# facebookresearch/dmc-net

Hardware: AMD Instinct MI355X
Metric: clips/sec (3-seg 224x224) DMC-gen+ResNet-18 train step (higher is better)
Workload: dtype f32

## Files before the change

dmc-net_amd/csrc/conv_x3q.hip:

```cpp
#include "dmc_common.h"
#include "x3s_common.h"
#include <type_traits>
#include <utility>

using namespace dmc;
using namespace dmc::x3;

namespace {

constexpr int QBM = 256, QBN = 64;
constexpr int QWSLOT = 3 * QBN * 32;
constexpr int QWB = 3 * QWSLOT;
constexpr int QEP = 272, QETILE = 32 * QEP;

template <int NW_, int NPB_, int NT_>
struct QG {
    static constexpr int NW = NW_, NPB = NPB_, NT = NT_;
    static constexpr int NA = NW / 2;
    static constexpr int KP = (NT + NA - 1) / NA;
    static constexpr int PT = 3 * KP;
    static constexpr int KW = (18 + NA - 1) / NA;
    static constexpr int ZROW = 32 * NT;
    static constexpr int PSL = (ZROW + 1) * 32;
    static constexpr int PB = 3 * PSL;
// ... 129 lines not shown
#pragma unroll
        for (int j = 0; j < TN; ++j)
#pragma unroll
            for (int e = 0; e < 16; ++e) acc[s][j][e] = 0.f;

    lds_cptr const L = (lds_cptr)lds_q;
    struct Frag { u32x4 X[3], W[TN][3]; };
    auto load_frags = [&](Frag& f, int xa, int wa, auto kc) {
        constexpr int k = decltype(kc)::value;
#pragma unroll
        for (int s = 0; s < 3; ++s) {
#pragma unroll
            for (int j = 0; j < TN; ++j)
                f.W[j][s] = *reinterpret_cast<const __attribute__((address_space(3))) u32x4*>(L + wa + ((k * 3 + s) * QBN + 32 * j) * 32);
            f.X[s] = *reinterpret_cast<const __attribute__((address_space(3))) u32x4*>(L + xa + s * QPSL);
        }
    };
    auto mfma_slot = [&](const Frag& f, auto ac, auto&& between) {
        constexpr int A = decltype(ac)::value;
#pragma unroll
        for (int p = 0; p < 6; ++p) {
            constexpr int WS[6] = {0, 0, 0, 1, 1, 2}, XS[6] = {2, 1, 0, 1, 0, 0};
#pragma unroll
            for (int j = 0; j < TN; ++j) acc[A][j] = mfma_bf16(f.W[j][WS[p]], f.X[XS[p]], acc[A][j]);
            between(p);
        }
    };
    auto nothing = [](int) {};
    constexpr int NRD = 3 + 3 * TN, NMF = 6 * TN;
    auto interleave = [&]() {
#pragma unroll
        for (int k = 0; k < (NRD < NMF ? NRD : NMF); ++k) {
            __builtin_amdgcn_sched_group_barrier(0x008, 1, 0);
            __builtin_amdgcn_sched_group_barrier(0x100, 1, 0);
        }
        if constexpr (NMF > NRD) __builtin_amdgcn_sched_group_barrier(0x008, NMF - NRD, 0);
    };

    if (tid < 2 * 3 * QNPB)
        *reinterpret_cast<float4*>(lds_q + (tid >> 1) / 3 * QPB + ((tid >> 1) % 3) * QPSL + QZROW * 32 + (tid & 1) * 16) = make_float4(0.f, 0.f, 0.f, 0.f);
    if (grp_a) {
        static_for<QNPB>([&](auto uc) {
            constexpr int U = decltype(uc)::value;
            if (U < total_units) {
#pragma unroll
                for (int i = 0; i < QPT; ++i) dma_patch(U / NUNIT, std::integral_constant<int, U % NUNIT>{}, U, i);
            }
// ... 54 lines not shown
            constexpr int kl = nslot - 1;
            constexpr int sh_first = P::STEP[JN].s[0].sh, acc_last = P::STEP[J].s[kl].acc;
            if (g + 1 < total_steps)
                load_frags(frag_of(std::integral_constant<int, (par + kl + 1) & 1>{}), xcur[sh_first], wcur, std::integral_constant<int, 0>{});
            constexpr int J2 = (J + 2) % NSTEP, C2 = (J + 2) / NSTEP;
            constexpr int U3 = (unit + QNPB) % NUNIT, CU3 = (unit + QNPB) / NUNIT;
            const bool wgo = !grp_a && g + 2 < total_steps;
            const bool pgo = grp_a && unit_last && U + QNPB < total_units;
            mfma_slot(frag_of(std::integral_constant<int, (par + kl) & 1>{}), std::integral_constant<int, acc_last>{}, [&](int p) {
                if (wgo) {
#pragma unroll
                    for (int i = p; i < KW; i += 6) dma_weight(c + C2, std::integral_constant<int, J2>{}, wb_old, wq + NA * i);
                }
                if constexpr (unit_last) {
                    if (pgo) {
#pragma unroll
                        for (int i = p; i < QPT; i += 6) dma_patch(c + CU3, std::integral_constant<int, U3>{}, pb_old, i);
                    }
                }
            });
        });
    }

    __syncthreads();
    constexpr int CW = 32 * TN, LPR = CW / 4, RPI = 64 / LPR;
    char* etile = lds_q + wave * QETILE;
    const int mw0 = m0 + wm * 32;
    const int rbase = blockIdx.y * QBN + wn * CW;
    const bool ok = mw0 + l31 <= mlast;
#pragma unroll
    for (int A = 0; A < NACC; ++A) {
#pragma unroll
        for (int j = 0; j < TN; ++j)
#pragma unroll
            for (int g4 = 0; g4 < 4; ++g4) {
                float4 v = make_float4(acc[A][j][4 * g4], acc[A][j][4 * g4 + 1], acc[A][j][4 * g4 + 2], acc[A][j][4 * g4 + 3]);
                if (!ok) v = make_float4(0.f, 0.f, 0.f, 0.f);
                *reinterpret_cast<float4*>(etile + l31 * QEP + (32 * j + 8 * g4 + 4 * khalf) * 4) = v;
            }
        float* const yout = (NACC == 2 && A == 1) ? a.y1 : a.y0;
        if constexpr (EVAL) {
            const int c4 = rbase + (lane % LPR) * 4;
            const float* const st = A == 1 ? a.stats1 : a.stats0;
            const float4 mean = *reinterpret_cast<const float4*>(st + c4), istd = *reinterpret_cast<const float4*>(st + a.R + c4);
            const float4 gm = *reinterpret_cast<const float4*>((A == 1 ? a.gamma1 : a.gamma0) + c4);
            const float4 bt = *reinterpret_cast<const float4*>((A == 1 ? a.beta1 : a.beta0) + c4);
            unsigned short* const ys = A == 1 ? nullptr : a.ys0;
#pragma unroll
            for (int it = 0; it < 32 / RPI; ++it) {
                const int prow = RPI * it + lane / LPR;
                const int m = mw0 + prow;
                const float4 v = *reinterpret_cast<const float4*>(etile + prow * QEP + (lane % LPR) * 16);
                if (m <= mlast) {
                    const float w[4] = {bn_apply_act1(v.x, mean.x, istd.x, gm.x, bt.x, false, 0.f, A == 0),
                                        bn_apply_act1(v.y, mean.y, istd.y, gm.y, bt.y, false, 0.f, A == 0),
                                        bn_apply_act1(v.z, mean.z, istd.z, gm.z, bt.z, false, 0.f, A == 0),
                                        bn_apply_act1(v.w, mean.w, istd.w, gm.w, bt.w, false, 0.f, A == 0)};
                    if (yout) *reinterpret_cast<float4*>(yout + (size_t)m * a.R + c4) = make_float4(w[0], w[1], w[2], w[3]);
                    if (ys) x3s_store4(ys, w, (size_t)a.M, a.R >> 4, (size_t)m, c4 >> 2);
                }
            }
        } else {
#pragma unroll
        for (int it = 0; it < 32 / RPI; ++it) {
            const int prow = RPI * it + lane / LPR;
            const int m = mw0 + prow;
            const float4 v = *reinterpret_cast<const float4*>(etile + prow * QEP + (lane % LPR) * 16);
            if (m <= mlast) {
                size_t opix = (size_t)m;
                if (NACC == 4) {
                    const int n = m / HW, rem = m - n * HW, ya = rem / a.W, xb = rem - ya * a.W;
                    opix = ((size_t)n * (2 * a.H) + 2 * ya + (A >> 1)) * (2 * a.W) + 2 * xb + (A & 1);
                }
                *reinterpret_cast<float4*>(yout + opix * a.R + rbase + (lane % LPR) * 4) = v;
            }
        }
        }
        if (NACC == 2 && !EVAL) {
            double* const part = A == 1 ? a.part1 : a.part0;
            if (part) {
                double* red = reinterpret_cast<double*>(lds_q + QNW * QETILE);
                if (lane < CW) {
                    double d1 = 0.0, d2 = 0.0;
#pragma unroll 8
                    for (int p = 0; p < 32; ++p) {
                        const double v = (double)*reinterpret_cast<const float*>(etile + p * QEP + lane * 4);
                        d1 += v;
                        d2 += v * v;
                    }
                    red[(wm * 64 + wn * CW + lane) * 2 + 0] = d1;
                    red[(wm * 64 + wn * CW + lane) * 2 + 1] = d2;
                }
                __syncthreads();
                for (int cc = tid; cc < QBN; cc += QNW * 64) {
                    double e1 = 0.0, e2 = 0.0;
#pragma unroll
                    for (int w = 0; w < WM; ++w) { e1 += red[(w * 64 + cc) * 2 + 0]; e2 += red[(w * 64 + cc) * 2 + 1]; }
                    double* dst = part + ((size_t)blockIdx.x * a.R + blockIdx.y * QBN + cc) * 2;
                    dst[0] = e1; dst[1] = e2;
                }
                __syncthreads();
            }
        }
    }
}

__global__ __launch_bounds__(256) void x3q_pack_w_kernel(const float* __restrict__ w3, const float* __restrict__ w1,
                                                         unsigned short* __restrict__ wf, unsigned short* __restrict__ wt, int Cout, int Cin) {
    const bool transposed = blockIdx.y == 1;
    unsigned short* dst = transposed ? wt : wf;
    if (!dst) return;
    const int R = transposed ? Cin : Cout, K = transposed ? Cout : Cin;
    const int nchunk = K >> 4;
    const long total = (long)R * 10 * K;
    for (long i = (long)blockIdx.x * 256 + threadIdx.x; i < total; i += (long)gridDim.x * 256) {
        long t = i;
        const int kk = (int)(t & 15); t >>= 4;
        const int rl = (int)(t & 63); t >>= 6;
        const int slot = (int)(t % 10); t /= 10;
        const int ch = (int)(t % nchunk);
        const int rt = (int)(t / nchunk);
        const int r = rt * 64 + rl, k = ch * 16 + kk;
        constexpr int FWD_TAP[10] = {0, 2, 6, 8, 3, 5, 1, 7, 4, 9};
        const int tap = transposed ? slot : FWD_TAP[slot];
// ... 550 lines not shown
```

dmc-net_amd/csrc/conv_x3s.hip:

```cpp
#include "dmc_common.h"
#include "x3s_common.h"
#include <type_traits>

using namespace dmc;
using namespace dmc::x3;

namespace {

__global__ __launch_bounds__(256) void x3s_split_kernel(const float* __restrict__ x, unsigned short* __restrict__ xs, long M, int C) {
    const int c8 = C >> 3;
    const long total = M * c8;
    const int nchunk = C >> 4;
    for (long o = (long)blockIdx.x * 256 + threadIdx.x; o < total; o += (long)gridDim.x * 256) {
        const long m = o / c8;
        const int g = (int)(o - m * c8);
        const float4 a = reinterpret_cast<const float4*>(x)[2 * o], b = reinterpret_cast<const float4*>(x)[2 * o + 1];
        const float v[8] = {a.x, a.y, a.z, a.w, b.x, b.y, b.z, b.w};
        x3s_store8(xs, v, (size_t)M, nchunk, (size_t)m, g);
    }
}

__global__ __launch_bounds__(256) void x3s_merge_kernel(const unsigned short* __restrict__ xs, float* __restrict__ x, long M, int C) {
    const long total = M * C;
    const size_t plane = (size_t)M * 16;
// ... 50 lines not shown
    const float* bnb_beta = nullptr;
    const unsigned char* bnb_mask = nullptr;
    int bnb_relu = 0;
    double* bnb_part = nullptr;
    int part_blocks = -1;
    int ablate;
    int bms = 0;
};
struct X3EvalArgs : X3Args {
    const float* stats;
    const float* gamma;
    const float* beta;
    const float* res;
    unsigned short* ys;
    int s2d, relu;
};

template <int WM, int WN, int TM, int TN, int PPMAX, bool STAG = false, int CLS = 1, bool EVAL = false, bool ROWT = false>
__global__ __launch_bounds__(WM * WN * 64) void x3s_conv_kernel(std::conditional_t<EVAL, X3EvalArgs, X3Args> a) {
    static_assert(!EVAL || CLS == 1, "the eval epilogue belongs to the forward convolution");
    static_assert(!ROWT || CLS == 1, "row-aligned tiles: forward and stride-1 data gradient");
    constexpr int NW = WM * WN, BM = 32 * TM * WM, BN = 32 * TN * WN;
    static_assert(BN == 64, "packed weight image is 64 rows wide");
    static_assert(PPMAX % 32 == 0 || PPMAX % 32 == 1, "patch transfers move 32 pixel rows");
    constexpr int PSL = PPMAX * 32;
    constexpr int PB = 3 * PSL;
    constexpr int WB = 3 * 3 * BN * 32;
    constexpr int WOFF = 2 * PB;
    static_assert(!STAG || NW >= 4, "two transfer groups need four waves");
    constexpr int NA = STAG ? NW / 2 : NW, NB = NW - (STAG ? NA : 0);
    constexpr int NDW = (PPMAX / 32 + NA - 1) / NA;
    constexpr int NEW = WB / 1024;
    constexpr int NEWW = (NEW + NB - 1) / NB;
    extern __shared__ __attribute__((aligned(1024))) char lds_x3[];

    const int tid = threadIdx.x, lane = tid & 63;
    const int wave = __builtin_amdgcn_readfirstlane(tid >> 6);
    const int wm = wave % WM, wn = wave / WM;
    const int l31 = lane & 31, khalf = lane >> 5;
    const unsigned lds0 = lds_addr_of(lds_x3);

    const int HW = a.H * a.W, PW = a.W;
    constexpr int ZROW = PPMAX - 1;
    const int bms = ROWT ? a.bms : BM;
    const int m0 = blockIdx.x * bms;
    const int mlast = (m0 + bms < a.M ? m0 + bms : a.M) - 1;
// ... 73 lines not shown
            xa[i] = xaddr[i][t];
            if constexpr (ROWT && pbuf == 1) asm volatile("" : "+v"(xa[i]));
        }
#pragma unroll
        for (int s = 0; s < 3; ++s) {
#pragma unroll
            for (int j = 0; j < TN; ++j)
                f.W[j][s] = *reinterpret_cast<const __attribute__((address_space(3))) u32x4*>(
                    L + waddr + (WOFF + wbuf * WB + (((t % 3) * 3 + s) * BN + 32 * j) * 32));
#pragma unroll
            for (int i = 0; i < TM; ++i)
                f.X[i][s] = *reinterpret_cast<const __attribute__((address_space(3))) u32x4*>(L + xa[i] + (pbuf * PB + s * PSL));
        }
    };
    auto mfma_frags = [&](const Frag& f, auto tc, auto&& between) {
        constexpr int t = decltype(tc)::value;
        constexpr int cl = CLS == 4 ? (t / 3 != 1) * 2 + (t % 3 != 1) : 0;
#pragma unroll
        for (int p = 0; p < 6; ++p) {
            constexpr int WS[6] = {0, 0, 0, 1, 1, 2}, XS[6] = {2, 1, 0, 1, 0, 0};
#pragma unroll
            for (int i = 0; i < TM; ++i)
#pragma unroll
                for (int j = 0; j < TN; ++j) acc[cl][i][j] = mfma_bf16(f.W[j][WS[p]], f.X[i][XS[p]], acc[cl][i][j]);
            between(p);
        }
    };
    auto nothing = [](int) {};
    constexpr int NRD = 3 * (TM + TN), NMF = 6 * TM * TN;
    auto interleave = [&]() {
#pragma unroll
        for (int k = 0; k < NRD; ++k) {
            __builtin_amdgcn_sched_group_barrier(0x008, 1, 0);
            __builtin_amdgcn_sched_group_barrier(0x100, 1, 0);
        }
        __builtin_amdgcn_sched_group_barrier(0x008, NMF - NRD, 0);
    };
    const bool dma_on = !(DMC_ABL(a.ablate) & 64);
    auto step = [&](auto pbufc, auto wbufc, auto qc, Frag& FA, Frag& FB, int c) {
        constexpr int pbuf = decltype(pbufc)::value, wbuf = decltype(wbufc)::value, q = decltype(qc)::value;
        using NP = std::integral_constant<int, q == 2 ? (pbuf ^ 1) : pbuf>;
        using NWB = std::integral_constant<int, wbuf ^ 1>;
        using NT = std::integral_constant<int, q == 2 ? 0 : 3 * (q + 1)>;
        using T0 = std::integral_constant<int, 3 * q>;
        using T1 = std::integral_constant<int, 3 * q + 1>;
        using T2 = std::integral_constant<int, 3 * q + 2>;
        const int s = 3 * c + q;
// ... 44 lines not shown
    if (tid < 12)
        *reinterpret_cast<float4*>(lds_x3 + (tid >> 1) * PSL + ZROW * 32 + (tid & 1) * 16) = make_float4(0.f, 0.f, 0.f, 0.f);
    issue_weights(0, 0);
    issue_patch(0, 0, 0); issue_patch(0, 1, 0); issue_patch(0, 2, 0);
    asm volatile("s_waitcnt vmcnt(0)" ::: "memory");
    __builtin_amdgcn_s_barrier();
    if (dma_on) {
        if (!STAG && S > 1) issue_weights(1, 1);
        if (nchunk > 1) issue_patch(1, 0, 1);
    }
    Frag F0, F1;
    load_frags(I0{}, I0{}, Q0{}, F0);
#pragma unroll 1
    for (int c = 0; c < ((DMC_ABL(a.ablate) & 256) ? 0 : nchunk); c += 2) {
        step(I0{}, I0{}, Q0{}, F0, F1, c);
        step(I0{}, I1{}, Q1{}, F1, F0, c);
        step(I0{}, I0{}, Q2{}, F0, F1, c);
        step(I1{}, I1{}, Q0{}, F1, F0, c + 1);
        step(I1{}, I0{}, Q1{}, F0, F1, c + 1);
        step(I1{}, I1{}, Q2{}, F1, F0, c + 1);
    }

    static_assert(WN == 1 && TN == 2, "epilogue: a wave owns all 64 channels of its pixels");
    constexpr int EP = 272, ETILE = 32 * TM * EP;
    char* etile = lds_x3 + wave * ETILE;
    const int mw0 = m0 + wm * TM * 32;
    const int rbase = blockIdx.y * BN;
    if constexpr (ROWT && !EVAL) {
        if (a.bnb_part) {
            constexpr int ET1 = 32 * EP;
            char* dtile = lds_x3 + wave * 2 * ET1;
            char* xtile = dtile + ET1;
            const int c4 = rbase + (lane & 15) * 4;
            const float4 mean = *reinterpret_cast<const float4*>(a.bnb_stats + c4);
            const float4 istd = *reinterpret_cast<const float4*>(a.bnb_stats + a.R + c4);
            double d1 = 0.0, d2 = 0.0;
#pragma unroll
            for (int i = 0; i < TM; ++i) {
                const bool ok = mw0 + 32 * i + l31 <= mlast;
#pragma unroll
                for (int j = 0; j < TN; ++j)
#pragma unroll
                    for (int g = 0; g < 4; ++g) {
                        float4 v = make_float4(acc[0][i][j][4 * g], acc[0][i][j][4 * g + 1], acc[0][i][j][4 * g + 2], acc[0][i][j][4 * g + 3]);
                        if (!ok) v = make_float4(0.f, 0.f, 0.f, 0.f);
                        *reinterpret_cast<float4*>(dtile + l31 * EP + (32 * j + 8 * g + 4 * khalf) * 4) = v;
                    }
#pragma unroll
                for (int it = 0; it < 8; ++it) {
                    const int prow = 4 * it + (lane >> 4);
                    const int m = mw0 + 32 * i + prow;
                    float4 v = *reinterpret_cast<const float4*>(dtile + prow * EP + (lane & 15) * 16);
                    float4 xh = make_float4(0.f, 0.f, 0.f, 0.f);
                    if (m <= mlast) {
                        const size_t o = (size_t)m * a.R + c4;
                        if (a.addend) {
                            const float4 av = *reinterpret_cast<const float4*>(a.addend + o);
                            v.x += av.x; v.y += av.y; v.z += av.z; v.w += av.w;
                        }
                        *reinterpret_cast<float4*>(a.y + o) = v;
                        const float4 yv = *reinterpret_cast<const float4*>(a.bnb_y + o);
                        xh = make_float4((yv.x - mean.x) * istd.x, (yv.y - mean.y) * istd.y, (yv.z - mean.z) * istd.z, (yv.w - mean.w) * istd.w);
                        if (a.bnb_relu) {
                            unsigned mb;
                            if (a.bnb_mask) {
                                mb = a.bnb_mask[o >> 2];
                            } else {
                                const float4 g = *reinterpret_cast<const float4*>(a.bnb_gamma + c4), b = *reinterpret_cast<const float4*>(a.bnb_beta + c4);
                                mb = (fmaf(xh.x, g.x, b.x) > 0.f ? 1u : 0u) | (fmaf(xh.y, g.y, b.y) > 0.f ? 2u : 0u) |
                                     (fmaf(xh.z, g.z, b.z) > 0.f ? 4u : 0u) | (fmaf(xh.w, g.w, b.w) > 0.f ? 8u : 0u);
                            }
                            v.x = (mb & 1) ? v.x : 0.f; v.y = (mb & 2) ? v.y : 0.f; v.z = (mb & 4) ? v.z : 0.f; v.w = (mb & 8) ? v.w : 0.f;
                        }
                    }
                    *reinterpret_cast<float4*>(dtile + prow * EP + (lane & 15) * 16) = v;
                    *reinterpret_cast<float4*>(xtile + prow * EP + (lane & 15) * 16) = xh;
                }
#pragma unroll 8
                for (int p = 0; p < 32; ++p) {
                    const double d = (double)*reinterpret_cast<const float*>(dtile + p * EP + lane * 4);
                    const double xh = (double)*reinterpret_cast<const float*>(xtile + p * EP + lane * 4);
                    d1 += d;
                    d2 += d * xh;
                }
            }
            double* red = reinterpret_cast<double*>(lds_x3 + NW * 2 * ET1);
            red[(wm * 64 + lane) * 2 + 0] = d1;
            red[(wm * 64 + lane) * 2 + 1] = d2;
            __syncthreads();
            for (int cc = tid; cc < BN; cc += NW * 64) {
                double e1 = 0.0, e2 = 0.0;
#pragma unroll
                for (int w = 0; w < WM; ++w) { e1 += red[(w * 64 + cc) * 2 + 0]; e2 += red[(w * 64 + cc) * 2 + 1]; }
                double* dst = a.bnb_part + ((size_t)blockIdx.x * a.R + rbase + cc) * 2;
                dst[0] = e1; dst[1] = e2;
            }
            return;
        }
    }
#pragma unroll
    for (int cl = 0; cl < CLS; ++cl) {
#pragma unroll
        for (int i = 0; i < TM; ++i) {
            const bool ok = mw0 + 32 * i + l31 <= mlast;
#pragma unroll
            for (int j = 0; j < TN; ++j)
#pragma unroll
                for (int g = 0; g < 4; ++g) {
                    float4 v = make_float4(acc[cl][i][j][4 * g], acc[cl][i][j][4 * g + 1], acc[cl][i][j][4 * g + 2], acc[cl][i][j][4 * g + 3]);
                    if (!ok) v = make_float4(0.f, 0.f, 0.f, 0.f);
                    *reinterpret_cast<float4*>(etile + (32 * i + l31) * EP + (32 * j + 8 * g + 4 * khalf) * 4) = v;
                }
        }
        if constexpr (EVAL) {
            const int c4 = rbase + (lane & 15) * 4;
            const float4 mean = *reinterpret_cast<const float4*>(a.stats + c4), istd = *reinterpret_cast<const float4*>(a.stats + a.R + c4);
            const float4 gm = *reinterpret_cast<const float4*>(a.gamma + c4), bt = *reinterpret_cast<const float4*>(a.beta + c4);
            const bool has_res = a.res != nullptr, relu = a.relu != 0;
            const int ochunk = a.R >> 4;
#pragma unroll
            for (int it = 0; it < 8 * TM; ++it) {
                const int prow = 4 * it + (lane >> 4);
                const int m = mw0 + prow;
                const float4 v = *reinterpret_cast<const float4*>(etile + prow * EP + (lane & 15) * 16);
                if (m <= mlast) {
                    const size_t o = (size_t)m * a.R + c4;
                    float4 rv = make_float4(0.f, 0.f, 0.f, 0.f);
                    if (has_res) rv = *reinterpret_cast<const float4*>(a.res + o);
                    const float w[4] = {bn_apply_act1(v.x, mean.x, istd.x, gm.x, bt.x, has_res, rv.x, relu),
                                        bn_apply_act1(v.y, mean.y, istd.y, gm.y, bt.y, has_res, rv.y, relu),
                                        bn_apply_act1(v.z, mean.z, istd.z, gm.z, bt.z, has_res, rv.z, relu),
                                        bn_apply_act1(v.w, mean.w, istd.w, gm.w, bt.w, has_res, rv.w, relu)};
                    if (a.y) *reinterpret_cast<float4*>(a.y + o) = make_float4(w[0], w[1], w[2], w[3]);
                    if (a.ys) {
                        if (a.s2d) {
                            const int n = m / HW, rem = m - n * HW, yy = rem / a.W, xx = rem - yy * a.W;
                            const int cls = (yy & 1) * 2 + (xx & 1);
                            const size_t mq = ((size_t)n * (a.H >> 1) + (yy >> 1)) * (a.W >> 1) + (xx >> 1);
                            x3s_store4(a.ys, w, (size_t)a.M >> 2, 4 * ochunk, mq, (c4 >> 2) + cls * 4 * ochunk);
                        } else {
                            x3s_store4(a.ys, w, (size_t)a.M, ochunk, (size_t)m, c4 >> 2);
                        }
                    }
                }
            }
        } else
        if (!(DMC_ABL(a.ablate) & 128)) {
#pragma unroll
            for (int it = 0; it < 8 * TM; ++it) {
                const int prow = 4 * it + (lane >> 4);
                const int m = mw0 + prow;
                float4 v = *reinterpret_cast<const float4*>(etile + prow * EP + (lane & 15) * 16);
                if (m <= mlast) {
                    size_t opix = (size_t)m;
                    if (CLS == 4) {
                        const int n = m / HW, rem = m - n * HW, ya = rem / a.W, xb = rem - ya * a.W;
                        opix = ((size_t)n * (2 * a.H) + 2 * ya + (cl >> 1)) * (2 * a.W) + 2 * xb + (cl & 1);
                    }
                    const size_t o = opix * a.R + rbase + (lane & 15) * 4;
                    if (a.addend) {
                        const float4 av = *reinterpret_cast<const float4*>(a.addend + o);
                        v.x += av.x; v.y += av.y; v.z += av.z; v.w += av.w;
                    }
                    *reinterpret_cast<float4*>(a.y + o) = v;
                    if (CLS == 1 && a.bnb_part) {
                        const int c4 = rbase + (lane & 15) * 4;
                        const float4 yv = *reinterpret_cast<const float4*>(a.bnb_y + o);
                        const float4 mean = *reinterpret_cast<const float4*>(a.bnb_stats + c4);
                        const float4 istd = *reinterpret_cast<const float4*>(a.bnb_stats + a.R + c4);
                        const float4 xh = make_float4((yv.x - mean.x) * istd.x, (yv.y - mean.y) * istd.y, (yv.z - mean.z) * istd.z, (yv.w - mean.w) * istd.w);
                        if (a.bnb_relu) {
                            unsigned mb;
                            if (a.bnb_mask) {
                                mb = a.bnb_mask[o >> 2];
                            } else {
                                const float4 g = *reinterpret_cast<const float4*>(a.bnb_gamma + c4), b = *reinterpret_cast<const float4*>(a.bnb_beta + c4);
                                mb = (fmaf(xh.x, g.x, b.x) > 0.f ? 1u : 0u) | (fmaf(xh.y, g.y, b.y) > 0.f ? 2u : 0u) |
                                     (fmaf(xh.z, g.z, b.z) > 0.f ? 4u : 0u) | (fmaf(xh.w, g.w, b.w) > 0.f ? 8u : 0u);
                            }
                            v.x = (mb & 1) ? v.x : 0.f; v.y = (mb & 2) ? v.y : 0.f; v.z = (mb & 4) ? v.z : 0.f; v.w = (mb & 8) ? v.w : 0.f;
                        }
                        *reinterpret_cast<float4*>(etile + prow * EP + (lane & 15) * 16) = v;
                        *reinterpret_cast<float4*>(etile + NW * ETILE + 8192 + prow * EP + (lane & 15) * 16) = xh;
                    }
                } else if (CLS == 1 && a.bnb_part) {
                    *reinterpret_cast<float4*>(etile + prow * EP + (lane & 15) * 16) = make_float4(0.f, 0.f, 0.f, 0.f);
                    *reinterpret_cast<float4*>(etile + NW * ETILE + 8192 + prow * EP + (lane & 15) * 16) = make_float4(0.f, 0.f, 0.f, 0.f);
                }
            }
        }
    }
    if constexpr (EVAL) return;
    if (CLS == 1 && a.bnb_part) {
        double* red = reinterpret_cast<double*>(lds_x3 + NW * ETILE);
        const char* xtile = etile + NW * ETILE + 8192;
        double d1 = 0.0, d2 = 0.0;
#pragma unroll 8
        for (int p = 0; p < 32 * TM; ++p) {
            const double d = (double)*reinterpret_cast<const float*>(etile + p * EP + lane * 4);
            const double xh = (double)*reinterpret_cast<const float*>(xtile + p * EP + lane * 4);
            d1 += d;
            d2 += d * xh;
        }
        red[(wm * 64 + lane) * 2 + 0] = d1;
        red[(wm * 64 + lane) * 2 + 1] = d2;
        __syncthreads();
        for (int cc = tid; cc < BN; cc += NW * 64) {
            double e1 = 0.0, e2 = 0.0;
#pragma unroll
            for (int w = 0; w < WM; ++w) { e1 += red[(w * 64 + cc) * 2 + 0]; e2 += red[(w * 64 + cc) * 2 + 1]; }
            double* dst = a.bnb_part + ((size_t)blockIdx.x * a.R + rbase + cc) * 2;
            dst[0] = e1; dst[1] = e2;
        }
    }
    if (CLS == 1 && a.stat_part) {
        double* red = reinterpret_cast<double*>(lds_x3 + NW * ETILE);
        double d1 = 0.0, d2 = 0.0;
#pragma unroll 8
        for (int p = 0; p < 32 * TM; ++p) {
            const double v = (double)*reinterpret_cast<const float*>(etile + p * EP + lane * 4);
            d1 += v;
            d2 += v * v;
        }
        red[(wm * 64 + lane) * 2 + 0] = d1;
        red[(wm * 64 + lane) * 2 + 1] = d2;
        __syncthreads();
        for (int c = tid; c < BN; c += NW * 64) {
            double e1 = 0.0, e2 = 0.0;
#pragma unroll
            for (int w = 0; w < WM; ++w) { e1 += red[(w * 64 + c) * 2 + 0]; e2 += red[(w * 64 + c) * 2 + 1]; }
            double* dst = a.stat_part + ((size_t)blockIdx.x * a.R + rbase + c) * 2;
            dst[0] = e1; dst[1] = e2;
        }
    }
}

int patch_pixels_max(int N, int H, int W, int BM) {
    const long M = (long)N * H * W;
    int worst = 0;
    long tiles = (M + BM - 1) / BM;
    if (tiles > W) tiles = W;
    for (long t = 0; t < tiles; ++t) {
        const long m0 = t * BM, ml = (m0 + BM < M ? m0 + BM : M) - 1;
        const long r0 = m0 / W, r1 = ml / W;
        const long f0 = (r0 > 0 ? r0 - 1 : 0) * W, f1 = (r1 + 2) * W;
        if ((int)(f1 - f0) + 1 > worst) worst = (int)(f1 - f0) + 1;
    }
    return worst;
}

struct X3Cfg { int id, BM, PPMAX, threads; };
constexpr X3Cfg X3CFGS[] = {{0, 256, 608, 512}, {1, 128, 320, 256}, {2, 64, 192, 128}, {3, 256, 608, 256}, {4, 128, 225, 256},
                            {5, 512, 640, 512}};

int x3s_tile_stride(int cfg, int W) { return cfg == 5 ? (W <= X3CFGS[5].BM ? (X3CFGS[5].BM / W) * W : 0) : X3CFGS[cfg].BM; }
// ... 12 lines not shown
    const long M = (long)N * H * W;
    const int forced = option(OPT_CONV_CFG);
    if (forced >= 101 && forced <= 105 && patch_pixels_max(N, H, W, X3CFGS[forced - 101].BM) <= X3CFGS[forced - 101].PPMAX) return forced - 101;
    if (forced == 107 && x3s_row_tiles_fit(W)) return 5;
    if (forced != 106 && patch_pixels_max(N, H, W, X3CFGS[4].BM) <= X3CFGS[4].PPMAX && ((M + X3CFGS[4].BM - 1) / X3CFGS[4].BM) * (R / 64) >= 512)
        return 4;
    if (forced != 108 && W == 56 && x3s_row_tiles_fit(W) && patch_pixels_max(N, H, W, X3CFGS[0].BM) <= X3CFGS[0].PPMAX) {
        const long r5 = (((M + x3s_tile_stride(5, W) - 1) / x3s_tile_stride(5, W)) * (R / 64) + 255) / 256;
        const long r0 = (((M + X3CFGS[0].BM - 1) / X3CFGS[0].BM) * (R / 64) + 255) / 256;
        if (9 * r5 < 5 * r0) return 5;
    }
    int fallback = -1;
    for (const X3Cfg& c : X3CFGS) {
        if (c.id > 2 || patch_pixels_max(N, H, W, c.BM) > c.PPMAX) continue;
        const long wgs = ((M + c.BM - 1) / c.BM) * (R / 64);
        if (wgs >= 160) return c.id;
        fallback = c.id;
    }
    return fallback;
}

template <int WM, int TM, int PPMAX, bool ROWT = false>
int launch_x3s(const X3Args& a, hipStream_t s) {
    constexpr int BM = 32 * TM * WM;
    constexpr size_t op_bytes = 2 * 3 * PPMAX * 32 + 2 * 3 * 3 * 64 * 32, ep_bytes = (ROWT ? 1 : 2) * (size_t)BM * 272 + 8192;
    constexpr size_t lds_bytes = op_bytes > ep_bytes ? op_bytes : ep_bytes;
    static_assert(lds_bytes <= 160 * 1024 && (!ROWT || 2 * WM * 32 * 272 + 8192 <= lds_bytes), "the tiles exceed the LDS");
    dim3 grid((a.M + a.bms - 1) / a.bms, a.R / 64);
    if ((a.stat_part || a.bnb_part) && a.part_blocks >= 0 && (unsigned)a.part_blocks != grid.x)
        return fail(DMC_E_INVALID, "x3s_conv: statistics partials have %d rows but this launch writes %u (dmc_x3s_conv_stat_blocks was "
                                   "called under another conv_cfg option?)", a.part_blocks, grid.x);
    if constexpr (WM >= 4) {
        if (ROWT || !(option(OPT_CONV_ABLATE) & 512)) {
            static LdsLimit lim_attr2;
    const hipError_t attr2 = lim_attr2.raise(reinterpret_cast<const void*>(&x3s_conv_kernel<WM, 1, TM, 2, PPMAX, true, 1, false, ROWT>), (int)lds_bytes);
            if (attr2 != hipSuccess) return fail(DMC_E_LAUNCH, "x3s_conv: cannot raise the dynamic LDS limit: %s", hipGetErrorString(attr2));
            x3s_conv_kernel<WM, 1, TM, 2, PPMAX, true, 1, false, ROWT><<<grid, WM * 64, lds_bytes, s>>>(a);
            return check_launch("x3s_conv");
        }
    }
    if constexpr (!ROWT) {
        static LdsLimit lim_attr;
        const hipError_t attr = lim_attr.raise(reinterpret_cast<const void*>(&x3s_conv_kernel<WM, 1, TM, 2, PPMAX>), (int)lds_bytes);
        if (attr != hipSuccess) return fail(DMC_E_LAUNCH, "x3s_conv: cannot raise the dynamic LDS limit: %s", hipGetErrorString(attr));
        x3s_conv_kernel<WM, 1, TM, 2, PPMAX><<<grid, WM * 64, lds_bytes, s>>>(a);
    }
    return check_launch("x3s_conv");
}

struct X3Bnb { const float *y, *stats, *gamma, *beta; const unsigned char* mask; int relu; double* part; };
// ... 420 lines not shown
```

Baseline: 3650.

## Store conv outputs straight from MFMA registers and reduce BN stats in registers

For the training (non-EVAL) paths of the x3s and x3q conv kernels, the MFMA operands are swapped so each lane holds one output channel across pixel rows. Accumulators are then written directly to global memory with buffer stores, using out-of-bounds offsets to mask rows past the tile end, instead of being staged through an LDS tile. BN statistics and the fused bnb partial sums are accumulated in registers and reduced with a cross-half shuffle and a small LDS buffer. This removes the LDS staging round trip and its barriers, and shrinks the LDS footprint. In exchange the global stores become per-lane 4-byte scattered writes rather than coalesced float4 rows.

```diff
diff --git a/dmc-net_amd/csrc/conv_x3q.hip b/dmc-net_amd/csrc/conv_x3q.hip
--- a/dmc-net_amd/csrc/conv_x3q.hip
+++ b/dmc-net_amd/csrc/conv_x3q.hip
@@ -175,7 +175,10 @@
         for (int p = 0; p < 6; ++p) {
             constexpr int WS[6] = {0, 0, 0, 1, 1, 2}, XS[6] = {2, 1, 0, 1, 0, 0};
 #pragma unroll
-            for (int j = 0; j < TN; ++j) acc[A][j] = mfma_bf16(f.W[j][WS[p]], f.X[XS[p]], acc[A][j]);
+            for (int j = 0; j < TN; ++j) {
+                if constexpr (EVAL) acc[A][j] = mfma_bf16(f.W[j][WS[p]], f.X[XS[p]], acc[A][j]);
+                else acc[A][j] = mfma_bf16(f.X[XS[p]], f.W[j][WS[p]], acc[A][j]);
+            }
             between(p);
         }
     };
@@ -276,24 +279,104 @@
         });
     }
 
-    __syncthreads();
-    constexpr int CW = 32 * TN, LPR = CW / 4, RPI = 64 / LPR;
-    char* etile = lds_q + wave * QETILE;
+    constexpr int CW = 32 * TN;
     const int mw0 = m0 + wm * 32;
     const int rbase = blockIdx.y * QBN + wn * CW;
-    const bool ok = mw0 + l31 <= mlast;
-#pragma unroll
-    for (int A = 0; A < NACC; ++A) {
-#pragma unroll
-        for (int j = 0; j < TN; ++j)
-#pragma unroll
-            for (int g4 = 0; g4 < 4; ++g4) {
-                float4 v = make_float4(acc[A][j][4 * g4], acc[A][j][4 * g4 + 1], acc[A][j][4 * g4 + 2], acc[A][j][4 * g4 + 3]);
-                if (!ok) v = make_float4(0.f, 0.f, 0.f, 0.f);
-                *reinterpret_cast<float4*>(etile + l31 * QEP + (32 * j + 8 * g4 + 4 * khalf) * 4) = v;
-            }
-        float* const yout = (NACC == 2 && A == 1) ? a.y1 : a.y0;
-        if constexpr (EVAL) {
+    if constexpr (!EVAL) {
+        const int plim = mlast - mw0 - 4 * khalf;
+        const int ch = rbase + l31;
+        auto in_tile = [&](int r) { return 8 * (r >> 2) + (r & 3) <= plim; };
+        unsigned voff[16];
+        if constexpr (NACC == 4) {
+#pragma unroll
+            for (int g = 0; g < 4; ++g) {
+                const int m = mw0 + 4 * khalf + 8 * g;
+                int n = m / HW, ya = (m - n * HW) / a.W, xb = m - n * HW - ya * a.W;
+#pragma unroll
+                for (int e = 0; e < 4; ++e) {
+                    const int opix = (n * 2 * a.H + 2 * ya) * 2 * a.W + 2 * xb;
+                    voff[4 * g + e] = in_tile(4 * g + e) ? (unsigned)(opix * a.R + ch) * 4u : OOB;
+                    if (++xb == a.W) {
+                        xb = 0;
+                        if (++ya == a.H) { ya = 0; ++n; }
+                    }
+                }
+            }
+        } else {
+            const unsigned lane_off = (unsigned)((mw0 + 4 * khalf) * a.R + ch) * 4u;
+#pragma unroll
+            for (int r = 0; r < 16; ++r) voff[r] = in_tile(r) ? lane_off : OOB;
+        }
+        auto soff = [&](int A, int r, int j) {
+            const int row = NACC == 4 ? (A >> 1) * 2 * a.W + (A & 1) : 8 * (r >> 2) + (r & 3);
+            return (row * a.R + 32 * j) * 4;
+        };
+        constexpr int NSET = NACC == 2 ? 2 : 1;
+        double s1[NSET][TN] = {}, s2[NSET][TN] = {};
+#pragma unroll
+        for (int A = 0; A < NACC; ++A) {
+            float* const yout = (NACC == 2 && A == 1) ? a.y1 : a.y0;
+            const __amdgpu_buffer_rsrc_t srd = __builtin_amdgcn_make_buffer_rsrc(yout, 0, 0x7fffffff, 0x00020000);
+            const bool stat = NACC == 2 && (A == 1 ? a.part1 : a.part0) != nullptr;
+#pragma unroll
+            for (int j = 0; j < TN; ++j) {
+#pragma unroll
+                for (int r = 0; r < 16; ++r)
+                    __builtin_amdgcn_raw_buffer_store_b32(__float_as_uint(acc[A][j][r]), srd, voff[r], soff(A, r, j), 0);
+                if (stat) {
+#pragma unroll
+                    for (int r = 0; r < 16; ++r) {
+                        const double w = (double)(in_tile(r) ? acc[A][j][r] : 0.f);
+                        s1[A % NSET][j] += w;
+                        s2[A % NSET][j] = fma(w, w, s2[A % NSET][j]);
+                    }
+                }
+            }
+        }
+        if (NACC == 2 && (a.part0 || a.part1)) {
+            __syncthreads();
+            double* red = reinterpret_cast<double*>(lds_q);
+#pragma unroll
+            for (int A = 0; A < NSET; ++A) {
+                const double g1 = __shfl_xor(TN == 2 && !khalf ? s1[A][TN - 1] : s1[A][0], 32, 64);
+                const double g2 = __shfl_xor(TN == 2 && !khalf ? s2[A][TN - 1] : s2[A][0], 32, 64);
+                const double k1 = TN == 2 && khalf ? s1[A][TN - 1] : s1[A][0], k2 = TN == 2 && khalf ? s2[A][TN - 1] : s2[A][0];
+                if (TN == 2 || !khalf) {
+                    double* dst = red + ((A * WM + wm) * 64 + wn * CW + (TN == 2 ? lane : l31)) * 2;
+                    dst[0] = khalf ? g1 + k1 : k1 + g1;
+                    dst[1] = khalf ? g2 + k2 : k2 + g2;
+                }
+            }
+            __syncthreads();
+#pragma unroll
+            for (int A = 0; A < NSET; ++A) {
+                double* const part = A == 1 ? a.part1 : a.part0;
+                if (!part) continue;
+                for (int cc = tid; cc < QBN; cc += QNW * 64) {
+                    double e1 = 0.0, e2 = 0.0;
+#pragma unroll
+                    for (int w = 0; w < WM; ++w) { e1 += red[((A * WM + w) * 64 + cc) * 2 + 0]; e2 += red[((A * WM + w) * 64 + cc) * 2 + 1]; }
+                    double* dst = part + ((size_t)blockIdx.x * a.R + blockIdx.y * QBN + cc) * 2;
+                    dst[0] = e1; dst[1] = e2;
+                }
+            }
+        }
+    } else {
+        __syncthreads();
+        constexpr int LPR = CW / 4, RPI = 64 / LPR;
+        char* etile = lds_q + wave * QETILE;
+        const bool ok = mw0 + l31 <= mlast;
+#pragma unroll
+        for (int A = 0; A < NACC; ++A) {
+#pragma unroll
+            for (int j = 0; j < TN; ++j)
+#pragma unroll
+                for (int g4 = 0; g4 < 4; ++g4) {
+                    float4 v = make_float4(acc[A][j][4 * g4], acc[A][j][4 * g4 + 1], acc[A][j][4 * g4 + 2], acc[A][j][4 * g4 + 3]);
+                    if (!ok) v = make_float4(0.f, 0.f, 0.f, 0.f);
+                    *reinterpret_cast<float4*>(etile + l31 * QEP + (32 * j + 8 * g4 + 4 * khalf) * 4) = v;
+                }
+            float* const yout = A == 1 ? a.y1 : a.y0;
             const int c4 = rbase + (lane % LPR) * 4;
             const float* const st = A == 1 ? a.stats1 : a.stats0;
             const float4 mean = *reinterpret_cast<const float4*>(st + c4), istd = *reinterpret_cast<const float4*>(st + a.R + c4);
@@ -313,47 +396,6 @@
                     if (yout) *reinterpret_cast<float4*>(yout + (size_t)m * a.R + c4) = make_float4(w[0], w[1], w[2], w[3]);
                     if (ys) x3s_store4(ys, w, (size_t)a.M, a.R >> 4, (size_t)m, c4 >> 2);
                 }
-            }
-        } else {
-#pragma unroll
-        for (int it = 0; it < 32 / RPI; ++it) {
-            const int prow = RPI * it + lane / LPR;
-            const int m = mw0 + prow;
-            const float4 v = *reinterpret_cast<const float4*>(etile + prow * QEP + (lane % LPR) * 16);
-            if (m <= mlast) {
-                size_t opix = (size_t)m;
-                if (NACC == 4) {
-                    const int n = m / HW, rem = m - n * HW, ya = rem / a.W, xb = rem - ya * a.W;
-                    opix = ((size_t)n * (2 * a.H) + 2 * ya + (A >> 1)) * (2 * a.W) + 2 * xb + (A & 1);
-                }
-                *reinterpret_cast<float4*>(yout + opix * a.R + rbase + (lane % LPR) * 4) = v;
-            }
-        }
-        }
-        if (NACC == 2 && !EVAL) {
-            double* const part = A == 1 ? a.part1 : a.part0;
-            if (part) {
-                double* red = reinterpret_cast<double*>(lds_q + QNW * QETILE);
-                if (lane < CW) {
-                    double d1 = 0.0, d2 = 0.0;
-#pragma unroll 8
-                    for (int p = 0; p < 32; ++p) {
-                        const double v = (double)*reinterpret_cast<const float*>(etile + p * QEP + lane * 4);
-                        d1 += v;
-                        d2 += v * v;
-                    }
-                    red[(wm * 64 + wn * CW + lane) * 2 + 0] = d1;
-                    red[(wm * 64 + wn * CW + lane) * 2 + 1] = d2;
-                }
-                __syncthreads();
-                for (int cc = tid; cc < QBN; cc += QNW * 64) {
-                    double e1 = 0.0, e2 = 0.0;
-#pragma unroll
-                    for (int w = 0; w < WM; ++w) { e1 += red[(w * 64 + cc) * 2 + 0]; e2 += red[(w * 64 + cc) * 2 + 1]; }
-                    double* dst = part + ((size_t)blockIdx.x * a.R + blockIdx.y * QBN + cc) * 2;
-                    dst[0] = e1; dst[1] = e2;
-                }
-                __syncthreads();
             }
         }
     }
diff --git a/dmc-net_amd/csrc/conv_x3s.hip b/dmc-net_amd/csrc/conv_x3s.hip
--- a/dmc-net_amd/csrc/conv_x3s.hip
+++ b/dmc-net_amd/csrc/conv_x3s.hip
@@ -96,6 +96,7 @@
     static_assert(!ROWT || CLS == 1, "row-aligned tiles: forward and stride-1 data gradient");
     constexpr int NW = WM * WN, BM = 32 * TM * WM, BN = 32 * TN * WN;
     static_assert(BN == 64, "packed weight image is 64 rows wide");
+    constexpr bool REGEP = !EVAL;
     static_assert(PPMAX % 32 == 0 || PPMAX % 32 == 1, "patch transfers move 32 pixel rows");
     constexpr int PSL = PPMAX * 32;
     constexpr int PB = 3 * PSL;
@@ -215,7 +216,10 @@
 #pragma unroll
             for (int i = 0; i < TM; ++i)
 #pragma unroll
-                for (int j = 0; j < TN; ++j) acc[cl][i][j] = mfma_bf16(f.W[j][WS[p]], f.X[i][XS[p]], acc[cl][i][j]);
+                for (int j = 0; j < TN; ++j) {
+                    if constexpr (REGEP) acc[cl][i][j] = mfma_bf16(f.X[i][XS[p]], f.W[j][WS[p]], acc[cl][i][j]);
+                    else acc[cl][i][j] = mfma_bf16(f.W[j][WS[p]], f.X[i][XS[p]], acc[cl][i][j]);
+                }
             between(p);
         }
     };
@@ -306,84 +310,131 @@
     }
 
     static_assert(WN == 1 && TN == 2, "epilogue: a wave owns all 64 channels of its pixels");
-    constexpr int EP = 272, ETILE = 32 * TM * EP;
-    char* etile = lds_x3 + wave * ETILE;
     const int mw0 = m0 + wm * TM * 32;
     const int rbase = blockIdx.y * BN;
-    if constexpr (ROWT && !EVAL) {
-        if (a.bnb_part) {
-            constexpr int ET1 = 32 * EP;
-            char* dtile = lds_x3 + wave * 2 * ET1;
-            char* xtile = dtile + ET1;
-            const int c4 = rbase + (lane & 15) * 4;
-            const float4 mean = *reinterpret_cast<const float4*>(a.bnb_stats + c4);
-            const float4 istd = *reinterpret_cast<const float4*>(a.bnb_stats + a.R + c4);
-            double d1 = 0.0, d2 = 0.0;
-#pragma unroll
-            for (int i = 0; i < TM; ++i) {
-                const bool ok = mw0 + 32 * i + l31 <= mlast;
-#pragma unroll
-                for (int j = 0; j < TN; ++j)
-#pragma unroll
-                    for (int g = 0; g < 4; ++g) {
-                        float4 v = make_float4(acc[0][i][j][4 * g], acc[0][i][j][4 * g + 1], acc[0][i][j][4 * g + 2], acc[0][i][j][4 * g + 3]);
-                        if (!ok) v = make_float4(0.f, 0.f, 0.f, 0.f);
-                        *reinterpret_cast<float4*>(dtile + l31 * EP + (32 * j + 8 * g + 4 * khalf) * 4) = v;
-                    }
-#pragma unroll
-                for (int it = 0; it < 8; ++it) {
-                    const int prow = 4 * it + (lane >> 4);
-                    const int m = mw0 + 32 * i + prow;
-                    float4 v = *reinterpret_cast<const float4*>(dtile + prow * EP + (lane & 15) * 16);
-                    float4 xh = make_float4(0.f, 0.f, 0.f, 0.f);
-                    if (m <= mlast) {
-                        const size_t o = (size_t)m * a.R + c4;
-                        if (a.addend) {
-                            const float4 av = *reinterpret_cast<const float4*>(a.addend + o);
-                            v.x += av.x; v.y += av.y; v.z += av.z; v.w += av.w;
-                        }
-                        *reinterpret_cast<float4*>(a.y + o) = v;
-                        const float4 yv = *reinterpret_cast<const float4*>(a.bnb_y + o);
-                        xh = make_float4((yv.x - mean.x) * istd.x, (yv.y - mean.y) * istd.y, (yv.z - mean.z) * istd.z, (yv.w - mean.w) * istd.w);
-                        if (a.bnb_relu) {
-                            unsigned mb;
-                            if (a.bnb_mask) {
-                                mb = a.bnb_mask[o >> 2];
-                            } else {
-                                const float4 g = *reinterpret_cast<const float4*>(a.bnb_gamma + c4), b = *reinterpret_cast<const float4*>(a.bnb_beta + c4);
-                                mb = (fmaf(xh.x, g.x, b.x) > 0.f ? 1u : 0u) | (fmaf(xh.y, g.y, b.y) > 0.f ? 2u : 0u) |
-                                     (fmaf(xh.z, g.z, b.z) > 0.f ? 4u : 0u) | (fmaf(xh.w, g.w, b.w) > 0.f ? 8u : 0u);
-                            }
-                            v.x = (mb & 1) ? v.x : 0.f; v.y = (mb & 2) ? v.y : 0.f; v.z = (mb & 4) ? v.z : 0.f; v.w = (mb & 8) ? v.w : 0.f;
+    if constexpr (REGEP) {
+        const int plim = mlast - mw0 - 4 * khalf;
+        const int ch = rbase + l31;
+        auto in_tile = [&](int i, int r) { return 32 * i + 8 * (r >> 2) + (r & 3) <= plim; };
+        unsigned voff[TM][16];
+        size_t base = 0;
+        if constexpr (CLS == 4) {
+            const int n0 = m0 / HW, ya0 = (m0 - n0 * HW) / a.W;
+            const int row0 = (n0 * 2 * a.H + 2 * ya0) * 2 * a.W;
+            base = (size_t)row0 * a.R;
+#pragma unroll
+            for (int i = 0; i < TM; ++i)
+#pragma unroll
+                for (int g = 0; g < 4; ++g) {
+                    const int m = mw0 + 4 * khalf + 32 * i + 8 * g;
+                    int n = m / HW, ya = (m - n * HW) / a.W, xb = m - n * HW - ya * a.W;
+#pragma unroll
+                    for (int e = 0; e < 4; ++e) {
+                        const int opix = (n * 2 * a.H + 2 * ya) * 2 * a.W + 2 * xb - row0;
+                        voff[i][4 * g + e] = in_tile(i, 4 * g + e) ? (unsigned)(opix * a.R + ch) * 4u : OOB;
+                        if (++xb == a.W) {
+                            xb = 0;
+                            if (++ya == a.H) { ya = 0; ++n; }
                         }
                     }
-                    *reinterpret_cast<float4*>(dtile + prow * EP + (lane & 15) * 16) = v;
-                    *reinterpret_cast<float4*>(xtile + prow * EP + (lane & 15) * 16) = xh;
                 }
-#pragma unroll 8
-                for (int p = 0; p < 32; ++p) {
-                    const double d = (double)*reinterpret_cast<const float*>(dtile + p * EP + lane * 4);
-                    const double xh = (double)*reinterpret_cast<const float*>(xtile + p * EP + lane * 4);
-                    d1 += d;
-                    d2 += d * xh;
+        } else {
+            const unsigned lane_off = (unsigned)((mw0 + 4 * khalf) * a.R + ch) * 4u;
+#pragma unroll
+            for (int i = 0; i < TM; ++i)
+#pragma unroll
+                for (int r = 0; r < 16; ++r) voff[i][r] = in_tile(i, r) ? lane_off : OOB;
+        }
+        auto soff = [&](int cl, int i, int r, int j) {
+            const int row = CLS == 4 ? (cl >> 1) * 2 * a.W + (cl & 1) : 32 * i + 8 * (r >> 2) + (r & 3);
+            return (row * a.R + 32 * j) * 4;
+        };
+        auto rsrc = [](const void* p) { return __builtin_amdgcn_make_buffer_rsrc(const_cast<void*>(p), 0, 0x7fffffff, 0x00020000); };
+        const bool stat = CLS == 1 && a.stat_part != nullptr, link = CLS == 1 && a.bnb_part != nullptr;
+        const __amdgpu_buffer_rsrc_t srd_y = rsrc(a.y + base), srd_add = rsrc(a.addend ? a.addend + base : nullptr);
+        const bool relu = link && a.bnb_relu, bymask = relu && a.bnb_mask != nullptr;
+        const __amdgpu_buffer_rsrc_t srd_by = rsrc(a.bnb_y), srd_mk = rsrc(a.bnb_mask);
+        float mean[TN] = {}, istd[TN] = {}, gm[TN] = {}, bt[TN] = {};
+        if (link) {
+#pragma unroll
+            for (int j = 0; j < TN; ++j) {
+                mean[j] = a.bnb_stats[ch + 32 * j]; istd[j] = a.bnb_stats[a.R + ch + 32 * j];
+                gm[j] = a.bnb_gamma[ch + 32 * j]; bt[j] = a.bnb_beta[ch + 32 * j];
+            }
+        }
+        double s1[TN] = {}, s2[TN] = {}, b1[TN] = {}, b2[TN] = {};
+#pragma unroll
+        for (int cl = 0; cl < CLS; ++cl)
+#pragma unroll
+            for (int i = 0; i < TM; ++i)
+#pragma unroll
+                for (int j = 0; j < TN; ++j) {
+                    float v[16];
+#pragma unroll
+                    for (int r = 0; r < 16; ++r) v[r] = acc[cl][i][j][r];
+                    if (stat) {
+#pragma unroll
+                        for (int r = 0; r < 16; ++r) {
+                            const double w = (double)(in_tile(i, r) ? v[r] : 0.f);
+                            s1[j] += w;
+                            s2[j] = fma(w, w, s2[j]);
+                        }
+                    }
+                    if (a.addend) {
+                        float av[16];
+#pragma unroll
+                        for (int r = 0; r < 16; ++r)
+                            av[r] = __uint_as_float(__builtin_amdgcn_raw_buffer_load_b32(srd_add, voff[i][r], soff(cl, i, r, j), 0));
+#pragma unroll
+                        for (int r = 0; r < 16; ++r) v[r] += av[r];
+                    }
+                    if (!(DMC_ABL(a.ablate) & 128)) {
+#pragma unroll
+                        for (int r = 0; r < 16; ++r)
+                            __builtin_amdgcn_raw_buffer_store_b32(__float_as_uint(v[r]), srd_y, voff[i][r], soff(cl, i, r, j), 0);
+                    }
+                    if (link) {
+                        float yv[16];
+                        unsigned mb[16] = {};
+#pragma unroll
+                        for (int r = 0; r < 16; ++r)
+                            yv[r] = __uint_as_float(__builtin_amdgcn_raw_buffer_load_b32(srd_by, voff[i][r], soff(cl, i, r, j), 0));
+                        if (bymask) {
+#pragma unroll
+                            for (int r = 0; r < 16; ++r)
+                                mb[r] = __builtin_amdgcn_raw_buffer_load_b8(srd_mk, in_tile(i, r) ? voff[i][r] >> 4 : OOB, soff(cl, i, r, j) >> 4, 0);
+                        }
+#pragma unroll
+                        for (int r = 0; r < 16; ++r) {
+                            const float xh = (yv[r] - mean[j]) * istd[j];
+                            bool on = in_tile(i, r);
+                            if (relu) on = on && (bymask ? ((mb[r] >> (l31 & 3)) & 1u) != 0u : fmaf(xh, gm[j], bt[j]) > 0.f);
+                            const double d = (double)(on ? v[r] : 0.f);
+                            b1[j] += d;
+                            b2[j] = fma(d, (double)(on ? xh : 0.f), b2[j]);
+                        }
+                    }
                 }
-            }
-            double* red = reinterpret_cast<double*>(lds_x3 + NW * 2 * ET1);
-            red[(wm * 64 + lane) * 2 + 0] = d1;
-            red[(wm * 64 + lane) * 2 + 1] = d2;
+        double* red = reinterpret_cast<double*>(lds_x3);
+        auto reduce_out = [&](const double (&t1)[TN], const double (&t2)[TN], double* part) {
+            const double g1 = __shfl_xor(khalf ? t1[0] : t1[1], 32, 64), g2 = __shfl_xor(khalf ? t2[0] : t2[1], 32, 64);
+            red[(wm * 64 + lane) * 2 + 0] = khalf ? g1 + t1[1] : t1[0] + g1;
+            red[(wm * 64 + lane) * 2 + 1] = khalf ? g2 + t2[1] : t2[0] + g2;
             __syncthreads();
-            for (int cc = tid; cc < BN; cc += NW * 64) {
+            for (int c = tid; c < BN; c += NW * 64) {
                 double e1 = 0.0, e2 = 0.0;
 #pragma unroll
-                for (int w = 0; w < WM; ++w) { e1 += red[(w * 64 + cc) * 2 + 0]; e2 += red[(w * 64 + cc) * 2 + 1]; }
-                double* dst = a.bnb_part + ((size_t)blockIdx.x * a.R + rbase + cc) * 2;
+                for (int w = 0; w < WM; ++w) { e1 += red[(w * 64 + c) * 2 + 0]; e2 += red[(w * 64 + c) * 2 + 1]; }
+                double* dst = part + ((size_t)blockIdx.x * a.R + rbase + c) * 2;
                 dst[0] = e1; dst[1] = e2;
             }
-            return;
-        }
-    }
-#pragma unroll
-    for (int cl = 0; cl < CLS; ++cl) {
+        };
+        if (link) reduce_out(b1, b2, a.bnb_part);
+        if (link && stat) __syncthreads();
+        if (stat) reduce_out(s1, s2, a.stat_part);
+    } else {
+        constexpr int EP = 272, ETILE = 32 * TM * EP;
+        char* etile = lds_x3 + wave * ETILE;
 #pragma unroll
         for (int i = 0; i < TM; ++i) {
             const bool ok = mw0 + 32 * i + l31 <= mlast;
@@ -391,130 +442,41 @@
             for (int j = 0; j < TN; ++j)
 #pragma unroll
                 for (int g = 0; g < 4; ++g) {
-                    float4 v = make_float4(acc[cl][i][j][4 * g], acc[cl][i][j][4 * g + 1], acc[cl][i][j][4 * g + 2], acc[cl][i][j][4 * g + 3]);
+                    float4 v = make_float4(acc[0][i][j][4 * g], acc[0][i][j][4 * g + 1], acc[0][i][j][4 * g + 2], acc[0][i][j][4 * g + 3]);
                     if (!ok) v = make_float4(0.f, 0.f, 0.f, 0.f);
                     *reinterpret_cast<float4*>(etile + (32 * i + l31) * EP + (32 * j + 8 * g + 4 * khalf) * 4) = v;
                 }
         }
-        if constexpr (EVAL) {
-            const int c4 = rbase + (lane & 15) * 4;
-            const float4 mean = *reinterpret_cast<const float4*>(a.stats + c4), istd = *reinterpret_cast<const float4*>(a.stats + a.R + c4);
-            const float4 gm = *reinterpret_cast<const float4*>(a.gamma + c4), bt = *reinterpret_cast<const float4*>(a.beta + c4);
-            const bool has_res = a.res != nullptr, relu = a.relu != 0;
-            const int ochunk = a.R >> 4;
-#pragma unroll
-            for (int it = 0; it < 8 * TM; ++it) {
-                const int prow = 4 * it + (lane >> 4);
-                const int m = mw0 + prow;
-                const float4 v = *reinterpret_cast<const float4*>(etile + prow * EP + (lane & 15) * 16);
-                if (m <= mlast) {
-                    const size_t o = (size_t)m * a.R + c4;
-                    float4 rv = make_float4(0.f, 0.f, 0.f, 0.f);
-                    if (has_res) rv = *reinterpret_cast<const float4*>(a.res + o);
-                    const float w[4] = {bn_apply_act1(v.x, mean.x, istd.x, gm.x, bt.x, has_res, rv.x, relu),
-                                        bn_apply_act1(v.y, mean.y, istd.y, gm.y, bt.y, has_res, rv.y, relu),
-                                        bn_apply_act1(v.z, mean.z, istd.z, gm.z, bt.z, has_res, rv.z, relu),
-                                        bn_apply_act1(v.w, mean.w, istd.w, gm.w, bt.w, has_res, rv.w, relu)};
-                    if (a.y) *reinterpret_cast<float4*>(a.y + o) = make_float4(w[0], w[1], w[2], w[3]);
-                    if (a.ys) {
-                        if (a.s2d) {
-                            const int n = m / HW, rem = m - n * HW, yy = rem / a.W, xx = rem - yy * a.W;
-                            const int cls = (yy & 1) * 2 + (xx & 1);
-                            const size_t mq = ((size_t)n * (a.H >> 1) + (yy >> 1)) * (a.W >> 1) + (xx >> 1);
-                            x3s_store4(a.ys, w, (size_t)a.M >> 2, 4 * ochunk, mq, (c4 >> 2) + cls * 4 * ochunk);
-                        } else {
-                            x3s_store4(a.ys, w, (size_t)a.M, ochunk, (size_t)m, c4 >> 2);
-                        }
+        const int c4 = rbase + (lane & 15) * 4;
+        const float4 mean = *reinterpret_cast<const float4*>(a.stats + c4), istd = *reinterpret_cast<const float4*>(a.stats + a.R + c4);
+        const float4 gm = *reinterpret_cast<const float4*>(a.gamma + c4), bt = *reinterpret_cast<const float4*>(a.beta + c4);
+        const bool has_res = a.res != nullptr, relu = a.relu != 0;
+        const int ochunk = a.R >> 4;
+#pragma unroll
+        for (int it = 0; it < 8 * TM; ++it) {
+            const int prow = 4 * it + (lane >> 4);
+            const int m = mw0 + prow;
+            const float4 v = *reinterpret_cast<const float4*>(etile + prow * EP + (lane & 15) * 16);
+            if (m <= mlast) {
+                const size_t o = (size_t)m * a.R + c4;
+                float4 rv = make_float4(0.f, 0.f, 0.f, 0.f);
+                if (has_res) rv = *reinterpret_cast<const float4*>(a.res + o);
+                const float w[4] = {bn_apply_act1(v.x, mean.x, istd.x, gm.x, bt.x, has_res, rv.x, relu),
+                                    bn_apply_act1(v.y, mean.y, istd.y, gm.y, bt.y, has_res, rv.y, relu),
+                                    bn_apply_act1(v.z, mean.z, istd.z, gm.z, bt.z, has_res, rv.z, relu),
+                                    bn_apply_act1(v.w, mean.w, istd.w, gm.w, bt.w, has_res, rv.w, relu)};
+                if (a.y) *reinterpret_cast<float4*>(a.y + o) = make_float4(w[0], w[1], w[2], w[3]);
+                if (a.ys) {
+                    if (a.s2d) {
+                        const int n = m / HW, rem = m - n * HW, yy = rem / a.W, xx = rem - yy * a.W;
+                        const int cls = (yy & 1) * 2 + (xx & 1);
+                        const size_t mq = ((size_t)n * (a.H >> 1) + (yy >> 1)) * (a.W >> 1) + (xx >> 1);
+                        x3s_store4(a.ys, w, (size_t)a.M >> 2, 4 * ochunk, mq, (c4 >> 2) + cls * 4 * ochunk);
+                    } else {
+                        x3s_store4(a.ys, w, (size_t)a.M, ochunk, (size_t)m, c4 >> 2);
                     }
                 }
             }
-        } else
-        if (!(DMC_ABL(a.ablate) & 128)) {
-#pragma unroll
-            for (int it = 0; it < 8 * TM; ++it) {
-                const int prow = 4 * it + (lane >> 4);
-                const int m = mw0 + prow;
-                float4 v = *reinterpret_cast<const float4*>(etile + prow * EP + (lane & 15) * 16);
-                if (m <= mlast) {
-                    size_t opix = (size_t)m;
-                    if (CLS == 4) {
-                        const int n = m / HW, rem = m - n * HW, ya = rem / a.W, xb = rem - ya * a.W;
-                        opix = ((size_t)n * (2 * a.H) + 2 * ya + (cl >> 1)) * (2 * a.W) + 2 * xb + (cl & 1);
-                    }
-                    const size_t o = opix * a.R + rbase + (lane & 15) * 4;
-                    if (a.addend) {
-                        const float4 av = *reinterpret_cast<const float4*>(a.addend + o);
-                        v.x += av.x; v.y += av.y; v.z += av.z; v.w += av.w;
-                    }
-                    *reinterpret_cast<float4*>(a.y + o) = v;
-                    if (CLS == 1 && a.bnb_part) {
-                        const int c4 = rbase + (lane & 15) * 4;
-                        const float4 yv = *reinterpret_cast<const float4*>(a.bnb_y + o);
-                        const float4 mean = *reinterpret_cast<const float4*>(a.bnb_stats + c4);
-                        const float4 istd = *reinterpret_cast<const float4*>(a.bnb_stats + a.R + c4);
-                        const float4 xh = make_float4((yv.x - mean.x) * istd.x, (yv.y - mean.y) * istd.y, (yv.z - mean.z) * istd.z, (yv.w - mean.w) * istd.w);
-                        if (a.bnb_relu) {
-                            unsigned mb;
-                            if (a.bnb_mask) {
-                                mb = a.bnb_mask[o >> 2];
-                            } else {
-                                const float4 g = *reinterpret_cast<const float4*>(a.bnb_gamma + c4), b = *reinterpret_cast<const float4*>(a.bnb_beta + c4);
-                                mb = (fmaf(xh.x, g.x, b.x) > 0.f ? 1u : 0u) | (fmaf(xh.y, g.y, b.y) > 0.f ? 2u : 0u) |
-                                     (fmaf(xh.z, g.z, b.z) > 0.f ? 4u : 0u) | (fmaf(xh.w, g.w, b.w) > 0.f ? 8u : 0u);
-                            }
-                            v.x = (mb & 1) ? v.x : 0.f; v.y = (mb & 2) ? v.y : 0.f; v.z = (mb & 4) ? v.z : 0.f; v.w = (mb & 8) ? v.w : 0.f;
-                        }
-                        *reinterpret_cast<float4*>(etile + prow * EP + (lane & 15) * 16) = v;
-                        *reinterpret_cast<float4*>(etile + NW * ETILE + 8192 + prow * EP + (lane & 15) * 16) = xh;
-                    }
-                } else if (CLS == 1 && a.bnb_part) {
-                    *reinterpret_cast<float4*>(etile + prow * EP + (lane & 15) * 16) = make_float4(0.f, 0.f, 0.f, 0.f);
-                    *reinterpret_cast<float4*>(etile + NW * ETILE + 8192 + prow * EP + (lane & 15) * 16) = make_float4(0.f, 0.f, 0.f, 0.f);
-                }
-            }
-        }
-    }
-    if constexpr (EVAL) return;
-    if (CLS == 1 && a.bnb_part) {
-        double* red = reinterpret_cast<double*>(lds_x3 + NW * ETILE);
-        const char* xtile = etile + NW * ETILE + 8192;
-        double d1 = 0.0, d2 = 0.0;
-#pragma unroll 8
-        for (int p = 0; p < 32 * TM; ++p) {
-            const double d = (double)*reinterpret_cast<const float*>(etile + p * EP + lane * 4);
-            const double xh = (double)*reinterpret_cast<const float*>(xtile + p * EP + lane * 4);
-            d1 += d;
-            d2 += d * xh;
-        }
-        red[(wm * 64 + lane) * 2 + 0] = d1;
-        red[(wm * 64 + lane) * 2 + 1] = d2;
-        __syncthreads();
-        for (int cc = tid; cc < BN; cc += NW * 64) {
-            double e1 = 0.0, e2 = 0.0;
-#pragma unroll
-            for (int w = 0; w < WM; ++w) { e1 += red[(w * 64 + cc) * 2 + 0]; e2 += red[(w * 64 + cc) * 2 + 1]; }
-            double* dst = a.bnb_part + ((size_t)blockIdx.x * a.R + rbase + cc) * 2;
-            dst[0] = e1; dst[1] = e2;
-        }
-    }
-    if (CLS == 1 && a.stat_part) {
-        double* red = reinterpret_cast<double*>(lds_x3 + NW * ETILE);
-        double d1 = 0.0, d2 = 0.0;
-#pragma unroll 8
-        for (int p = 0; p < 32 * TM; ++p) {
-            const double v = (double)*reinterpret_cast<const float*>(etile + p * EP + lane * 4);
-            d1 += v;
-            d2 += v * v;
-        }
-        red[(wm * 64 + lane) * 2 + 0] = d1;
-        red[(wm * 64 + lane) * 2 + 1] = d2;
-        __syncthreads();
-        for (int c = tid; c < BN; c += NW * 64) {
-            double e1 = 0.0, e2 = 0.0;
-#pragma unroll
-            for (int w = 0; w < WM; ++w) { e1 += red[(w * 64 + c) * 2 + 0]; e2 += red[(w * 64 + c) * 2 + 1]; }
-            double* dst = a.stat_part + ((size_t)blockIdx.x * a.R + rbase + c) * 2;
-            dst[0] = e1; dst[1] = e2;
         }
     }
 }
@@ -573,10 +535,8 @@
 
 template <int WM, int TM, int PPMAX, bool ROWT = false>
 int launch_x3s(const X3Args& a, hipStream_t s) {
-    constexpr int BM = 32 * TM * WM;
-    constexpr size_t op_bytes = 2 * 3 * PPMAX * 32 + 2 * 3 * 3 * 64 * 32, ep_bytes = (ROWT ? 1 : 2) * (size_t)BM * 272 + 8192;
-    constexpr size_t lds_bytes = op_bytes > ep_bytes ? op_bytes : ep_bytes;
-    static_assert(lds_bytes <= 160 * 1024 && (!ROWT || 2 * WM * 32 * 272 + 8192 <= lds_bytes), "the tiles exceed the LDS");
+    constexpr size_t lds_bytes = 2 * 3 * PPMAX * 32 + 2 * 3 * 3 * 64 * 32, ep_bytes = (size_t)WM * 64 * 2 * sizeof(double);
+    static_assert(ep_bytes <= lds_bytes && lds_bytes <= 160 * 1024, "the tiles exceed the LDS");
     dim3 grid((a.M + a.bms - 1) / a.bms, a.R / 64);
     if ((a.stat_part || a.bnb_part) && a.part_blocks >= 0 && (unsigned)a.part_blocks != grid.x)
         return fail(DMC_E_INVALID, "x3s_conv: statistics partials have %d rows but this launch writes %u (dmc_x3s_conv_stat_blocks was "
```

Result: no change. 3677, median of 6 (+0.7%).
